# tomneda/DABstar

Hardware: AMD Instinct MI355X
Metric: DAB Mode-I ensembles/s (2.048 MS/s IQ->MSC bytes) per GPU; FIB CRC match % (higher is better)
Workload: dtype f32+i32

## Files before the change

dabstar_amd/csrc/engine.cpp:

```cpp
#include "engine.h"
#include "viterbi_core.h"
#include "fig00.h"
#include <algorithm>
#include <cstddef>
#include <cstring>
#include <map>
#include <string>
#include <tuple>
#include <vector>

int dabx_engine::build_msc_classes()
{
  const EngineDev &d = dev;
  have_fast = false;
  fast = MscFast{};
  for (void *q : fast_allocs) {
    (void)hipFree(q);
    allocs.erase(std::remove(allocs.begin(), allocs.end(), q), allocs.end());
  }
  fast_allocs.clear();
  for (auto &sc : subch_host) sc.fast_class = 0;
  if (d.max_subch <= 0) return 0;
  struct Key { int kbps, prot, shortf, cu; bool operator<(const Key &o) const { return std::tie(kbps, prot, shortf, cu) < std::tie(o.kbps, o.prot, o.shortf, o.cu); } };
  std::map<Key, std::vector<uint32_t>> groups;
// ... 116 lines not shown
{
  if (!cfg || !out || cfg->n_streams <= 0 || cfg->ring_frames < 2 || cfg->max_subch < 0 || cfg->max_subch > MAX_SUBCH ||
      cfg->out_frames < 1 || cfg->soft_bit_type < 1 || cfg->soft_bit_type > 3 || cfg->dc_iq_correction < 0 || cfg->dc_iq_correction > 2 ||
      cfg->viterbi_tie_mode < 0 || cfg->viterbi_tie_mode > 2 || cfg->schedule < 0 || cfg->schedule > 1 ||
      cfg->msc_fast_min_jobs < 0 || cfg->msc_class_min_jobs < 0 || cfg->exact_level_tracker < 0 || cfg->exact_level_tracker > 2 ||
      cfg->acquire_mode < 0 || cfg->acquire_mode > 2) {
    set_error("dabx_create: bad configuration");
    return DABX_E_ARG;
  }
  int rc = need_device_e();
  if (rc) return rc;
  auto *e = new dabx_engine();
  e->cfg = *cfg;
#define H(x) do { hipError_t err__ = (x); if (err__ != hipSuccess) { set_error("HIP error %d (%s) at %s:%d", (int)err__, hipGetErrorString(err__), __FILE__, __LINE__); dabx_destroy(e); return DABX_E_HIP; } } while (0)
  H(hipGetDevice(&e->device));
  int prio_lo = 0, prio_hi = 0;
  (void)hipDeviceGetStreamPriorityRange(&prio_lo, &prio_hi);
  H(hipStreamCreateWithPriority(&e->stream, hipStreamNonBlocking, prio_hi));
  e->ss.a = e->stream;
  if (cfg->schedule == 0) {
    H(hipStreamCreateWithPriority(&e->ss.b, hipStreamNonBlocking, prio_lo));
    H(hipStreamCreateWithPriority(&e->ss.d, hipStreamNonBlocking, prio_hi));
    H(hipEventCreateWithFlags(&e->ss.prep_done, hipEventDisableTiming | hipEventReleaseToDevice));
    H(hipEventCreateWithFlags(&e->ss.msc_done, hipEventDisableTiming | hipEventReleaseToDevice));
    H(hipEventCreateWithFlags(&e->ss.fic_go, hipEventDisableTiming | hipEventReleaseToDevice));
    H(hipEventCreateWithFlags(&e->ss.prep_b_done, hipEventDisableTiming | hipEventReleaseToDevice));
    H(hipEventCreateWithFlags(&e->ss.demap_done, hipEventDisableTiming | hipEventReleaseToDevice));
    H(hipEventCreateWithFlags(&e->ss.sym_done, hipEventDisableTiming | hipEventReleaseToDevice));
    e->ss.fic_on_d = cfg->n_streams < FEW_STREAMS;
    H(hipStreamCreateWithFlags(&e->ingest, hipStreamNonBlocking));
        H(hipStreamCreateWithPriority(&e->ss.q, hipStreamNonBlocking, cfg->exact_level_tracker == 1 ? prio_hi : prio_lo));
    H(hipEventCreateWithFlags(&e->ss.acq_done, hipEventDisableTiming | hipEventReleaseToDevice));
    H(hipEventCreateWithFlags(&e->ss.tail_done, hipEventDisableTiming | hipEventReleaseToDevice));
    H(hipEventCreateWithFlags(&e->ss.acq_a_done, hipEventDisableTiming | hipEventReleaseToDevice));
  }
  if (!e->ingest) H(hipStreamCreateWithFlags(&e->ingest, hipStreamNonBlocking));
  H(hipEventCreateWithFlags(&e->ingest_done, hipEventDisableTiming | hipEventReleaseToDevice));
  e->rd_seen.assign(cfg->n_streams, 0);
  const int S = cfg->n_streams;
  EngineDev &d = e->dev;
  d.n_streams = S; d.max_subch = cfg->max_subch; d.out_frames = cfg->out_frames;
  d.ring_len = cfg->ring_frames * TF;
  d.ring_fmt = e->ring_fmt = ring_fmt;
  d.threshold = cfg->sync_threshold; d.strongest = cfg->sync_strongest;
  d.fic_only = cfg->fic_only; d.capture_soft = cfg->capture_soft; d.tie_mode = cfg->viterbi_tie_mode;
  d.exact_level = cfg->exact_level_tracker == 1;
  d.anchor_level = cfg->exact_level_tracker == 0;
  const DevTables *t;
  if ((rc = get_tables(&t))) { dabx_destroy(e); return rc; }
#define A(x) if ((rc = (x))) { dabx_destroy(e); return rc; }
  A(e->alloc_bytes(&d.iq, (size_t)S * d.ring_len * ring_bytes_per_sample(ring_fmt), false));
  A(e->alloc(&d.wr, S));
  A(e->alloc(&d.ctl, S));
  A(e->alloc(&d.spectra, (size_t)2 * S * 75 * K, false));
  A(e->alloc(&d.fsnap, S));
  A(e->alloc(&d.sym_seq, S));
  A(e->alloc(&d.fic_seq, S));
  A(e->alloc(&d.demap_busy, S));
  A(e->alloc(&d.dciq_state, (size_t)S * 8));
  A(e->alloc(&d.dciq_done, S));
  if (d.exact_level) A(e->alloc(&d.level_pos, S));
  H(hipHostMalloc((void **)&e->locked_host, sizeof(int32_t), hipHostMallocMapped | hipHostMallocCoherent));
  *e->locked_host = 0;
  H(hipHostMalloc((void **)&e->horizon_host, sizeof(unsigned long long) * S, hipHostMallocMapped | hipHostMallocCoherent));
  for (int s = 0; s < S; s++) e->horizon_host[s] = 0;
  e->announcing.assign(S, 0);
  H(hipHostGetDevicePointer((void **)&d.wr_horizon, e->horizon_host, 0));
  H(hipHostGetDevicePointer((void **)&d.locked_count, e->locked_host, 0));
  H(hipHostMalloc((void **)&e->seq_timeouts_host, sizeof(int32_t), hipHostMallocMapped | hipHostMallocCoherent));
  *e->seq_timeouts_host = 0;
  H(hipHostGetDevicePointer((void **)&d.seq_timeouts, e->seq_timeouts_host, 0));
  {
    std::vector<float> st8((size_t)S * 8, 0.0f);
    for (int s_ = 0; s_ < S; s_++) { st8[(size_t)s_ * 8 + 2] = 1.0f; st8[(size_t)s_ * 8 + 3] = 1.0f; }
    H(hipMemcpyAsync(d.dciq_state, st8.data(), sizeof(float) * st8.size(), hipMemcpyHostToDevice, e->stream));
    H(hipStreamSynchronize(e->stream));
  }
  A(e->alloc(&d.nco_tid, (size_t)S * 256));
  A(e->alloc(&d.nco_sym, (size_t)S * 76));
  A(e->alloc(&d.sym_off, (size_t)S * 76));
  A(e->alloc(&e->snap_buf[0], S));
  A(e->alloc(&e->snap_buf[1], S));
  d.snap = e->snap_buf[0];
  A(e->alloc(&d.tii_acc, (size_t)S * TU));
  A(e->alloc(&d.tii_cnt, (size_t)S * 2));
  e->tii.assign((size_t)S, nullptr);
  e->fibdec.assign((size_t)S, nullptr);
  e->fib_frames_fed.assign((size_t)S, 0);
  e->tii_epoch.assign((size_t)S, 0);
  A(e->alloc(&d.cp_part, (size_t)S * 75));
  A(e->alloc(&d.abs_part, (size_t)S * 76));
  A(e->alloc(&d.fic_sym, (size_t)S * 3 * K2));
  A(e->alloc(&d.tdi, (size_t)S * TDI_SLOTS * CIF_BITS));
  A(e->alloc(&d.subch, (size_t)S * std::max(1, d.max_subch)));
  A(e->alloc(&d.fib_out, (size_t)S * d.out_frames * 12 * 32));
  A(e->alloc(&d.fib_crc, (size_t)S * d.out_frames * 12));
  A(e->alloc(&d.frame_pos, (size_t)S * d.out_frames));
  A(e->alloc(&d.frame_start, (size_t)S * d.out_frames));
  if (d.capture_soft) A(e->alloc(&d.soft_cap, (size_t)S * 75 * K2));
  A(e->alloc(&d.sf_info, (size_t)S * std::max(1, d.max_subch) * SF_SLOTS));
  A(demap_alloc(d.demap, S));
  d.demap.soft_type = cfg->soft_bit_type;
  A(launch_demap_init(d.demap, e->stream));
  std::vector<StreamCtl> ctl(S);
  for (auto &c : ctl) {
    memset(&c, 0, sizeof(c));
    c.state = ST_INIT; c.s_level = 0.1f; c.peak_level = -1.0e6f; c.sync_thr = cfg->sync_threshold;
// ... 876 lines not shown
```

dabstar_amd/csrc/ofdm_core.h:

```cpp
#pragma once
#include <hip/hip_runtime.h>
#include "dabx_internal.h"
#include "fft_core.h"
#include "wave_ops.h"

namespace dabx {

__device__ __forceinline__ float cabsf_(float2 z) { return sqrtf(z.x * z.x + z.y * z.y); }
__device__ __forceinline__ float cabsf_level(float2 z) { return __builtin_amdgcn_sqrtf(z.x * z.x + z.y * z.y); }

__device__ __forceinline__ float block_sum(float v, float *red , int tid)
{
  v = wave_sum(v);
  __syncthreads();
  if ((tid & 63) == 0) red[tid >> 6] = v;
  __syncthreads();
  const int nw = blockDim.x >> 6;
  float s = 0.f;
  for (int w = 0; w < nw; w++) s += red[w];
  return s;
}
__device__ __forceinline__ void block_sum2(float &a, float &b, float *red , int tid)
{
  a = wave_sum(a); b = wave_sum(b);
// ... 295 lines not shown
  const float at_axis = mean_level * F_SQRT1_2;
  const float rd = fabsf(b.x) - at_axis, id = fabsf(b.y) - at_axis;
  const float sigma_sq = rd * rd + id * id;
  c.mean_sigma_sq += ALPHA * (sigma_sq - c.mean_sigma_sq);
  float signal_power = c.mean_power - c.null_power;
  if (signal_power <= 0.0f) signal_power = 0.1f;
  const float babs = __builtin_amdgcn_sqrtf(power);
  const float nsr = c.null_power * __builtin_amdgcn_rcpf(signal_power) + 0.7f;
  float w1;
  if (soft_type == 3) {
    w1 = pr_abs;
  } else if (soft_type == 2) {
    w1 = pr_abs * __builtin_amdgcn_rcpf(c.mean_sigma_sq * nsr);
  } else {
    w1 = __builtin_amdgcn_sqrtf(babs * pr_abs) * mean_level * __builtin_amdgcn_rcpf(nsr * (c.mean_sigma_sq * babs));
  }
  const float2 r1 = make_float2(b.x * w1, b.y * w1);
  soft_re = cvt_i16_x86(r1.x * w2);
  soft_im = cvt_i16_x86(r1.y * w2);
  c.prev = x;
  return babs * w1;
}

typedef float v2f __attribute__((ext_vector_type(2)));
typedef int v2i __attribute__((ext_vector_type(2)));
struct DemapPair {
  v2f prev_re, prev_im, integ, mean_power, mean_sigma_sq, null_power;
};
__device__ __forceinline__ v2f v2_rsq(v2f a) { return (v2f){__builtin_amdgcn_rsqf(a.x), __builtin_amdgcn_rsqf(a.y)}; }
__device__ __forceinline__ v2f v2_sqrt(v2f a) { return (v2f){__builtin_amdgcn_sqrtf(a.x), __builtin_amdgcn_sqrtf(a.y)}; }
__device__ __forceinline__ v2f v2_rcp(v2f a) { return (v2f){__builtin_amdgcn_rcpf(a.x), __builtin_amdgcn_rcpf(a.y)}; }
__device__ __forceinline__ v2f v2_abs(v2f a) { return (v2f){fabsf(a.x), fabsf(a.y)}; }
__device__ __forceinline__ v2f v2_fma(v2f a, v2f b, v2f c) { return __builtin_elementwise_fma(a, b, c); }

__device__ __forceinline__ v2f phase_offset_from_diagonal2(v2f y, v2f x, v2f ay, v2f ax)
{
  const v2f mx = (v2f){max3_abs(x.x, y.x, 1.17549435e-38f), max3_abs(x.y, y.y, 1.17549435e-38f)};
  const v2f mnv = (v2f){min_abs(x.x, y.x), min_abs(x.y, y.y)};
  const v2f t = mnv * v2_rcp(mx);
  const v2f z = t * t;
  v2f p = (v2f)(0.0028662257f);
  p = v2_fma(p, z, (v2f)(-0.0161657367f));
  p = v2_fma(p, z, (v2f)(0.0429096138f));
  p = v2_fma(p, z, (v2f)(-0.0752896400f));
  p = v2_fma(p, z, (v2f)(0.1065626393f));
  p = v2_fma(p, z, (v2f)(-0.1420889944f));
  p = v2_fma(p, z, (v2f)(0.1999355085f));
  p = v2_fma(p, z, (v2f)(-0.3333314528f));
  const v2f r = v2_fma(p * z, t, t);
  const v2f u = r - 0.78539816339744830962f, d = ay - ax;
  return (v2f){phase_fold_sign(u.x, d.x, x.x, y.x, t.x), phase_fold_sign(u.y, d.y, x.y, y.y, t.y)};
}

template <int SOFT_TYPE>
__device__ __forceinline__ v2f demap_pair(DemapPair &c, v2f x_re, v2f x_im, v2f rel_f, float clock_err, float w2,
                                          int16_t (&soft_re)[2], int16_t (&soft_im)[2], v2f &power_out, v2f *std_dev_sq = nullptr)
{
  constexpr float ALPHA = 0.005f;
  const float F_PI = 3.14159265358979323846f;
  const float F_RAD_PER_DEG = 0.01745329251994329577f, F_SQRT1_2 = 0.70710678118654752440f;
  const v2f pr_re = c.prev_re, pr_im = c.prev_im;
  const v2f pr_sq = pr_re * pr_re + pr_im * pr_im;
  const v2f pr_inv = v2_rsq(pr_sq);
  const v2f pr_abs = pr_sq * pr_inv;
  const v2f raw_re = (x_re * pr_re + x_im * pr_im) * pr_inv;
  const v2f raw_im = (x_im * pr_re - x_re * pr_im) * pr_inv;
  const v2f phase_err = clock_err * (F_PI / 1024.0f / (float)(K / 2)) * rel_f + c.integ;
  const v2f xx = -phase_err, x2 = xx * xx;
  const v2f sine = xx * (x2 * -0.16034401953220367431640625f + 0.99903142452239990234375f);
  const v2f cosine = 0.9994032382965087890625f + x2 * (x2 * 3.679168224334716796875e-2f + -0.495580852031707763671875f);
  const v2f b_re = raw_re * cosine - raw_im * sine;
  const v2f b_im = raw_re * sine + raw_im * cosine;
  const v2f abs_re = v2_abs(b_re), abs_im = v2_abs(b_im);
  const v2f off = phase_offset_from_diagonal2(b_im, b_re, abs_im, abs_re);
  const v2f integ = c.integ + 0.2f * ALPHA * off;
  const float lim = F_RAD_PER_DEG * 20.0f;
  c.integ = (v2f){__builtin_amdgcn_fmed3f(integ.x, -lim, lim), __builtin_amdgcn_fmed3f(integ.y, -lim, lim)};
  if (std_dev_sq) { v2f sd = *std_dev_sq; sd += ALPHA * (off * off - sd); *std_dev_sq = sd; }
  const v2f power = b_re * b_re + b_im * b_im;
  power_out = power;
  c.mean_power += ALPHA * (power - c.mean_power);
  const v2f mean_level = v2_sqrt(c.mean_power);
  const v2f at_axis = mean_level * F_SQRT1_2;
  const v2f rd = abs_re - at_axis, id = abs_im - at_axis;
  const v2f sigma_sq = rd * rd + id * id;
  c.mean_sigma_sq += ALPHA * (sigma_sq - c.mean_sigma_sq);
  v2f signal_power = c.mean_power - c.null_power;
  signal_power = (signal_power <= 0.0f) ? (v2f)(0.1f) : signal_power;
  const v2f babs = v2_sqrt(power);
  const v2f nsr = c.null_power * v2_rcp(signal_power) + 0.7f;
  v2f w1;
  if (SOFT_TYPE == 3) w1 = pr_abs;
  else if (SOFT_TYPE == 2) w1 = pr_abs * v2_rcp(c.mean_sigma_sq * nsr);
  else w1 = v2_sqrt(babs * pr_abs) * mean_level * v2_rcp(nsr * (c.mean_sigma_sq * babs));
  const v2f r1_re = b_re * w1, r1_im = b_im * w1;
  const v2f s_re = r1_re * w2, s_im = r1_im * w2;
  cvt4_i16_x86(s_re.x, s_re.y, s_im.x, s_im.y, soft_re[0], soft_re[1], soft_im[0], soft_im[1]);
  c.prev_re = x_re; c.prev_im = x_im;
  return babs * w1;
}

__device__ __forceinline__ float demap_w2(float mean_value, int soft_type)
{
  return (soft_type == 1 ? -100.0f : -140.0f) * __builtin_amdgcn_rcpf(mean_value);
}

__device__ __forceinline__ float mpa_weight(int k)
{
  const float a = 0.005f / (float)K;
  return a * __expf((float)(K - 1 - k) * -3.2552135e-6f);
}
__device__ __forceinline__ float mpa_decay() { return 0.99501247f; }
__device__ __forceinline__ float mpa_decay_n(int n_sym) { return __expf((float)n_sym * (float)K * -3.2552135e-6f); }
__device__ __forceinline__ float snr_db_from(float mean_power_all, float null_sum)
{
  const float kMinNoisePower = (1.0f / 32767.0f) * (1.0f / 32767.0f);
  if (null_sum == 0.0f) null_sum = kMinNoisePower * (float)K;
  const float noise = null_sum / (float)K;
  float snr = (mean_power_all - noise) / noise;
// ... 27 lines not shown
```

dabstar_amd/csrc/pipeline.h:

```cpp
#pragma once
#include "dabx_internal.h"
#include "ring_fmt.h"

namespace dabx {

#ifndef DABX_MSC_BATCH
#define DABX_MSC_BATCH 7
#endif
constexpr int MSC_SLOTS = DABX_MSC_BATCH > 7 ? 64 : 32;
constexpr int MSC_BATCH_FRAMES = DABX_MSC_BATCH;
constexpr int SF_SLOTS = 16;
constexpr int ACQ_NEED = 20 * TU + 50 + (TF + 1) + (TN + 50 + 21) + 64;
constexpr int FRAME_NEED = TF + 2 * TU;
constexpr int FEW_STREAMS = 48;

enum StreamState : int32_t { ST_INIT = 0, ST_WAIT_SYNC = 1, ST_EVAL_SYNC = 2 };

struct StreamCtl {
  unsigned long long rd;
  unsigned long long sym0_pos;
  long long cif_no;
  long long msc_done_cif;
  long long frames;
  int32_t state;
// ... 4 lines not shown
  float sync_thr;
  int32_t sample_count;
  int32_t start_index;
  int32_t correction;
  int32_t frame_ok;
  int32_t phase_sym1;
  int32_t f_frame;
  int32_t fic_ratio;
  int32_t cif_count;
  int32_t fic_errors, fic_bits, fic_block;
  int32_t fic_status_errors, fic_status_bits;
  float mer_db;
  float snr_db;
  long long fib_ok, fib_total, sync_lost;
  float head_abs_a, head_abs_b;
  int32_t np_sel;
  int32_t pad_;
  long long level_margin;
  unsigned long long lvl_anchor_pos, lvl_approx_pos;
  float lvl_anchor_S;
  int32_t pad3_;
  long long lvl_rewalks, lvl_unanchored;
  long long lvl_healed;
  unsigned long long lvl_hist_pos[16];
  float lvl_hist_S[16];
};
constexpr int LVL_HIST = 16;

struct SubchDev {
  int32_t cu_start, cu_size, kbps, prot_level, short_form, dab_plus;
  int32_t nbits;
  int32_t active;
  int32_t fast_class, pad_;
  const uint16_t *map;
  long long start_cif;
  long long cif_out;
  int32_t blocks_in_buf, sf_sync;
  long long sf_count;
  long long sf_ok, sf_fail, rs_corr, rs_fail, fc_corr, au_ok, au_bad;
  long long move_cif;
  int32_t prev_cu_start, pad2_;
};
#ifdef __HIPCC__
__device__ __forceinline__ int msc_move_thr(const SubchDev &sc, long long r)
{
  const long long t = sc.move_cif - r + 16;
  return t <= 0 ? 0 : (t >= 16 ? 16 : (int)t);
}
#endif

struct BatchSnap { long long msc_done, cif_no; };
struct FrameSnap { long long cif0; float clock_err; int32_t frame_ok, np_sel, pad_; };

struct EngineDev {
  int32_t n_streams, max_subch, out_frames;
  int32_t ring_len;
  float threshold;
  int32_t strongest, fic_only, capture_soft;
  int32_t exact_level;
  int32_t anchor_level;
  unsigned long long *wr_horizon;
  unsigned long long *level_pos;
  int32_t *locked_count;
  int32_t tie_mode;
  int32_t msc_stride;
  int32_t sf_stride;
  int32_t vit_stride;
  void *iq;
  int32_t ring_fmt;
  unsigned long long *wr;
  StreamCtl *ctl;
  DemapDev demap;
  float2 *spectra;
  FrameSnap *fsnap;
  int32_t *demap_busy;
  float *dciq_state;
  unsigned long long *dciq_done;
  int32_t parity;
  int32_t s0;
  int32_t flag_sync;
  uint32_t step_seq;
  uint32_t *sym_seq, *fic_seq;
  int32_t *seq_timeouts;
  double2 *nco_tid;
  double2 *nco_sym;
  int32_t *sym_off;
  float2 *cp_part;
  float *abs_part;
  uint8_t *fic_sym;
  uint8_t *tdi;
  uint32_t *vit_scratch;
  SubchDev *subch;
  uint8_t *fib_out;
  uint8_t *fib_crc;
  long long *frame_pos;
  int32_t *frame_start;
  uint8_t *msc_out;
  uint8_t *sf_out;
  dabx_superframe_info *sf_info;
  int16_t *soft_cap;
  BatchSnap *snap;
  float2 *tii_acc;
  int32_t *tii_cnt;
};

struct DeliverDev {
  uint8_t *slab;
  const unsigned long long *layout_off;
  const int32_t *subch_id;
  long long *frames_done;
  long long *cif_done, *sf_done;
  dabx_chunk_header hdr;
  hipEvent_t lf_done;
};

constexpr int MSC_MAX_CLASSES = DABX_MSC_FAST_CLASSES;
struct MscClass {
  int n_in, nbits;
  int n_pairs;
  const uint16_t *map2;
  const uint32_t *pairs;
  uint32_t *inT[2];
  uint2 *decT;
};
struct MscFast {
  int n_cls;
// ... 164 lines not shown
```

dabstar_amd/csrc/pipeline.hip:

```cpp
#include <type_traits>
#include "pipeline.h"
#include "packet_core.h"
#include "pad_core.h"
#include "mot_core.h"
#include "carousel_core.h"
#include <algorithm>
#include "ofdm_core.h"
#include "viterbi_core.h"
#include "fec_core.h"
#include "acq_walk.h"
#include "level_par.h"
#include "fig00.h"

namespace dabx {

__device__ __forceinline__ void front_prio() { __builtin_amdgcn_s_setprio(3); }

template <class T> __device__ __forceinline__ T uniform_load(const T *p)
{
  typedef unsigned Raw __attribute__((ext_vector_type(sizeof(T) / 4)));
  const Raw raw = *(const __attribute__((address_space(4))) Raw *)(const void *)p;
  return __builtin_bit_cast(T, raw);
}

// ... 724 lines not shown
  FftTwiddles tw;
  fft_load_twiddles(tw, t.twiddle, tid);
  const uint4 kk4 = reinterpret_cast<const uint4 *>(t.bin_to_slot8)[tid];
  const unsigned kkw[4] = {kk4.x, kk4.y, kk4.z, kk4.w};
  const unsigned rd_lo = t.carrier_slot_rd[tid];
  for (;;) {
    float2 cb0 = Fmt::cvt(nx[0]), ca0 = Fmt::cvt(nx[1]), cb1 = Fmt::cvt(nx[2]), ca1 = Fmt::cvt(nx[3]);
    float2 v[8];
#pragma unroll
    for (int u = 0; u < 8; u++) v[u] = Fmt::cvt(nx[4 + u]);
    const double2 base_now = nco_base;
    const int l_next = l + (int)gridDim.x;
    if (l_next < 75) {
      off = uniform_load(e.sym_off + (size_t)s * 76 + l_next);
      nco_base = uniform_load(e.nco_sym + (size_t)s * 76 + l_next);
      request(off);
    }
    asm volatile("" ::: "memory");
    float cre = 0.f, cim = 0.f, asum = 0.f;
    cre += ca0.x * cb0.x + ca0.y * cb0.y;
    cim += ca0.y * cb0.x - ca0.x * cb0.y;
    asum += cabsf_level(cb0);
    if (two) {
      cre += ca1.x * cb1.x + ca1.y * cb1.y;
      cim += ca1.y * cb1.x - ca1.x * cb1.y;
      asum += cabsf_level(cb1);
    }
    Nco nco;
    nco.init_from(base_now, nco_step, nco_t);
#pragma unroll
    for (int u = 0; u < 8; u++) {
      const float2 x = v[u];
      asum += cabsf_level(x);
      v[u] = nco.mix(x);
      nco.step();
    }
    cre = wave_sum(cre); cim = wave_sum(cim); asum = wave_sum(asum);
    if ((tid & 63) == 0) { red3[0][tid >> 6] = cre; red3[1][tid >> 6] = cim; red3[2][tid >> 6] = asum; }
    fft2048_regs<false>(v, lds, tw, tid);
    if (tid == 0) {
      float r[3];
#pragma unroll
      for (int q = 0; q < 3; q++) { float a = 0.f; for (int w = 0; w < 4; w++) a += red3[q][w]; r[q] = a; }
      e.cp_part[(size_t)s * 75 + l] = make_float2(r[0], r[1]); e.abs_part[(size_t)s * 76 + l] = r[2];
    }
#pragma unroll
    for (int u = 0; u < 8; u++) {
      unsigned kw = kkw[u >> 1];
      if (RF != RING_CF32) asm volatile("" : "+v"(kw));
      const int kk = (int)(int16_t)(kw >> (16 * (u & 1)));
      if (kk >= 0) lds[kk] = v[u];
    }
    __syncthreads();
    float2 *dst = e.spectra + (((size_t)e.parity * e.n_streams + s) * 75 + l) * K;
#pragma unroll
    for (int u = 0; u < K / 256; u++) {
      typedef float sym_f2 __attribute__((ext_vector_type(2)));
      const float2 q = lds[((tid + 256 * u) & ~15) | ((rd_lo >> (4 * u)) & 15u)];
      sym_f2 qv; qv.x = q.x; qv.y = q.y;
      __builtin_nontemporal_store(qv, reinterpret_cast<sym_f2 *>(dst + tid + 256 * u));
    }
    if (l_next >= 75) break;
    l = l_next;
    __syncthreads();
  }
}

__device__ __forceinline__ void seq_publish(uint32_t *p, uint32_t seq)
{
  __syncthreads();
  if (threadIdx.x == 0) {
    __threadfence();
    __hip_atomic_store(p, seq, __ATOMIC_RELEASE, __HIP_MEMORY_SCOPE_AGENT);
  }
}
__device__ __forceinline__ void seq_wait(const uint32_t *p, uint32_t seq, int32_t *timeouts)
{
  if (threadIdx.x == 0) {
    int spins = 0;
    while ((int32_t)(__hip_atomic_load(p, __ATOMIC_ACQUIRE, __HIP_MEMORY_SCOPE_AGENT) - seq) < 0) {
      __builtin_amdgcn_s_sleep(8);
      if (++spins > (8 << 20)) {
        if (timeouts) __hip_atomic_fetch_add(timeouts, 1, __ATOMIC_RELAXED, __HIP_MEMORY_SCOPE_SYSTEM);
        break;
      }
    }
  }
  __syncthreads();
  __builtin_amdgcn_fence(__ATOMIC_ACQUIRE, "agent");
}
__global__ void k_sym_publish(EngineDev e)
{
  const int s = blockIdx.x * blockDim.x + threadIdx.x;
  if (s < e.n_streams) __hip_atomic_store(e.sym_seq + s, e.step_seq, __ATOMIC_RELEASE, __HIP_MEMORY_SCOPE_AGENT);
}

constexpr int DEMAP_Q = 2, DEMAP_THREADS = K / DEMAP_Q, DEMAP_NP = DEMAP_Q / 2;
constexpr int DEMAP_NOUT = (K2 / 4) / DEMAP_THREADS;
constexpr int TILE_PLANE = 196;
__device__ __forceinline__ float2 demap_ld_spec(const float2 *p)
{
  typedef float dm_f2 __attribute__((ext_vector_type(2)));
  const dm_f2 q = __builtin_nontemporal_load(reinterpret_cast<const dm_f2 *>(p));
  return make_float2(q.x, q.y);
}
template <int SOFT_TYPE, bool SAT, bool WHOLE = false, bool MER = false>
__device__ __forceinline__ void demap_frame_body(EngineDev &e, const DevTables &t, const int l0, const int l1)
{
  if (l0 == 0) __builtin_amdgcn_s_setprio(3); else __builtin_amdgcn_s_setprio(1);
  __shared__ __attribute__((aligned(16))) float red[32];
  __shared__ __attribute__((aligned(16))) uint8_t tile[2][16 * TILE_PLANE];
  __shared__ v2f sd_lds[MER ? DEMAP_NP * DEMAP_THREADS : 1];
  const int s = blockIdx.x + e.s0, tid = threadIdx.x;
  StreamCtl &c = e.ctl[s];
  if (l0 == 0 && e.flag_sync) seq_wait(e.sym_seq + s, e.step_seq, e.seq_timeouts);
  FrameSnap fs;
  if (l0 == 0) {
    fs.cif0 = c.cif_no; fs.clock_err = c.clock_err; fs.frame_ok = c.frame_ok; fs.np_sel = c.np_sel; fs.pad_ = 0;
    if (tid == 0) {
      e.fsnap[s] = fs;
      if (fs.frame_ok && e.demap_busy) __hip_atomic_store(&e.demap_busy[s], 1, __ATOMIC_RELAXED, __HIP_MEMORY_SCOPE_AGENT);
    }
  } else fs = e.fsnap[s];
  if (!fs.frame_ok) {
    if (l0 == 0 && e.flag_sync) seq_publish(e.fic_seq + s, e.step_seq);
    return;
  }
  DemapDev &d = e.demap;
  const float *null_power = fs.np_sel ? d.null_power2 : d.null_power;
  const float2 *spectra = e.spectra + (size_t)e.parity * e.n_streams * 75 * K;
  DemapPair cr[DEMAP_NP];
  v2f rel_f[DEMAP_NP], wk[DEMAP_NP], pacc[DEMAP_NP];
#pragma unroll
  for (int q = 0; q < DEMAP_Q; q++) {
    const int k = tid + DEMAP_THREADS * q, p = q >> 1, h = q & 1;
    const int bin = t.perm_bin[k];
    rel_f[p][h] = (float)(K / 2 - t.perm_rel[k]);
    const float2 pr = l0 == 0 ? d.phase_ref[(size_t)s * TU + bin] : spectra[((size_t)s * 75 + (l0 - 1)) * K + k];
    cr[p].prev_re[h] = pr.x; cr[p].prev_im[h] = pr.y;
    cr[p].integ[h] = d.integ[(size_t)s * K + k];
    cr[p].mean_power[h] = d.mean_power[(size_t)s * K + k];
    cr[p].mean_sigma_sq[h] = d.mean_sigma[(size_t)s * K + k];
    cr[p].null_power[h] = null_power[(size_t)s * TU + bin];
    wk[p][h] = mpa_weight(k);
    pacc[p][h] = 0.0f;
    if constexpr (MER) sd_lds[p * DEMAP_THREADS + tid][h] = d.std_dev[(size_t)s * K + k];
  }
  float mean_value = d.mean_value[s], mpa = d.mean_power_all[s];
  const float ce = fs.clock_err;
  const long long cif0 = (long long)(((unsigned long long)(unsigned)__builtin_amdgcn_readfirstlane((int)((unsigned long long)fs.cif0 >> 32)) << 32) |
                                     (unsigned)__builtin_amdgcn_readfirstlane((int)(unsigned)fs.cif0));
  uint8_t *fic = e.fic_sym + (size_t)s * 3 * K2;
  uint8_t *tdi = e.tdi + (size_t)s * TDI_SLOTS * CIF_BITS;
  int16_t *cap = e.capture_soft ? e.soft_cap + (size_t)s * 75 * K2 : nullptr;
  float2 xn[DEMAP_Q];
  const float2 *xp = spectra + ((size_t)s * 75 + l0) * K + tid + (DEMAP_Q / 2) * DEMAP_THREADS;
#pragma unroll
  for (int q = 0; q < DEMAP_Q; q++) xn[q] = demap_ld_spec(xp + (q - DEMAP_Q / 2) * DEMAP_THREADS);
  static_assert(DEMAP_Q % 2 == 0 && K % DEMAP_Q == 0 && (K2 / 4) % DEMAP_THREADS == 0 && DEMAP_THREADS % 64 == 0, "tile <-> thread mapping below");
  int tpos[2 * DEMAP_Q];
#pragma unroll
  for (int q = 0; q < DEMAP_Q; q++) {
    const int k = tid + DEMAP_THREADS * q;
    tpos[2 * q] = (k & 15) * TILE_PLANE + (k >> 4);
    tpos[2 * q + 1] = ((K + k) & 15) * TILE_PLANE + ((K + k) >> 4);
  }
  auto symbol = [&](const int l, auto par) {
    constexpr int PAR = decltype(par)::value;
    if (l < 74) xp += K;
    const int m = l - 3, cif = m / 18, blk = m % 18;
    const float w2 = demap_w2(mean_value, SOFT_TYPE);
    uint8_t *tl = tile[PAR];
    float2 xc[DEMAP_Q];
#pragma unroll
    for (int q = 0; q < DEMAP_Q; q++) { xc[q] = xn[q]; xn[q] = demap_ld_spec(xp + (q - DEMAP_Q / 2) * DEMAP_THREADS); }
    float part = 0.f;
#pragma unroll
    for (int p = 0; p < DEMAP_NP; p++) {
      int16_t sr[2], si[2];
      v2f pw;
      const v2f mag = demap_pair<SOFT_TYPE>(cr[p], (v2f){xc[2 * p].x, xc[2 * p + 1].x}, (v2f){xc[2 * p].y, xc[2 * p + 1].y}, rel_f[p], ce, w2, sr, si, pw,
                                            MER ? &sd_lds[p * DEMAP_THREADS + tid] : nullptr);
      part = p == 0 ? mag.x + mag.y : part + (mag.x + mag.y);
      pacc[p] = pacc[p] * mpa_decay() + pw;
#pragma unroll
      for (int h = 0; h < 2; h++) {
        const int q = 2 * p + h;
        tl[tpos[2 * q]] = SAT ? soft_to_sym_sat(sr[h]) : soft_to_sym(sr[h]);
        tl[tpos[2 * q + 1]] = SAT ? soft_to_sym_sat(si[h]) : soft_to_sym(si[h]);
        if (cap) { const int k = tid + DEMAP_THREADS * q; cap[(size_t)l * K2 + k] = sr[h]; cap[(size_t)l * K2 + K + k] = si[h]; }
      }
    }
    {
      float *rp = red + 16 * PAR;
      const float pw_sum = wave_sum(part);
      if ((tid & 63) == 0) rp[tid >> 6] = pw_sum;
      __syncthreads();
      float sum = 0.f;
      if constexpr (DEMAP_THREADS / 64 == 12) {
        const v2f *rp2 = reinterpret_cast<const v2f *>(rp);
        const v2f a = ((rp2[0] + rp2[1]) + (rp2[2] + rp2[3])) + (rp2[4] + rp2[5]);
        sum = a.x + a.y;
      } else {
#pragma unroll
        for (int w = 0; w < DEMAP_THREADS / 64; w++) sum += rp[w];
      }
      mean_value = sum * (1.0f / (float)K);
    }
#pragma unroll
    for (int j = 0; j < DEMAP_NOUT; j++) {
      const int dwi = tid + DEMAP_THREADS * j;
      if (l < 3) {
        uint32_t v = 0;
#pragma unroll
        for (int b = 0; b < 4; b++) { const int i = 4 * dwi + b; v |= (uint32_t)tl[(i & 15) * TILE_PLANE + (i >> 4)] << (8 * b); }
        reinterpret_cast<uint32_t *>(fic + l * K2)[dwi] = v;
      } else {
        const int out_plane = dwi / 48, out_dw = dwi - out_plane * 48;
        const uint32_t v = *reinterpret_cast<const uint32_t *>(tl + out_plane * TILE_PLANE + 4 * out_dw);
        static_assert(K2 % 16 == 0, "a symbol is a whole number of positions in every plane");
        uint8_t *const tdi_thr = tdi + (size_t)out_plane * (CIF_BITS / 16) + 4 * out_dw;
        const size_t uoff = (size_t)((cif0 + cif) & (TDI_SLOTS - 1)) * CIF_BITS + (size_t)blk * (K2 / 16);
        *reinterpret_cast<uint32_t *>(tdi_thr + uoff) = v;
      }
    }
  };
  auto run = [&](int a, int b) {
    int l = a;
    for (; l + 1 < b; l += 2) { symbol(l, std::integral_constant<int, 0>{}); symbol(l + 1, std::integral_constant<int, 1>{}); }
    if (l < b) symbol(l, std::integral_constant<int, 0>{});
  };
  constexpr bool whole_frame_flagged = WHOLE;
  if constexpr (WHOLE) {
    run(0, 3);
    seq_publish(e.fic_seq + s, e.step_seq);
    run(3, l1);
  } else run(l0, l1);
#pragma unroll
  for (int q = 0; q < DEMAP_Q; q++) {
    const int k = tid + DEMAP_THREADS * q, p = q >> 1, h = q & 1;
    d.integ[(size_t)s * K + k] = cr[p].integ[h];
    d.mean_power[(size_t)s * K + k] = cr[p].mean_power[h];
    d.mean_sigma[(size_t)s * K + k] = cr[p].mean_sigma_sq[h];
  }
  if constexpr (MER) {
    float sd = 0.f;
#pragma unroll
    for (int q = 0; q < DEMAP_Q; q++) {
      const float v = sd_lds[(q >> 1) * DEMAP_THREADS + tid][q & 1];
      d.std_dev[(size_t)s * K + tid + DEMAP_THREADS * q] = v;
      sd += v;
    }
    if (l1 == 75) {
      sd = block_sum(sd, red, tid);
      if (tid == 0) c.mer_db = mer_db_from(sd);
      __syncthreads();
    }
  }
  float ns = cr[0].null_power.x + cr[0].null_power.y, wsum = wk[0].x * pacc[0].x + wk[0].y * pacc[0].y;
#pragma unroll
  for (int p = 1; p < DEMAP_NP; p++) { ns += cr[p].null_power.x + cr[p].null_power.y; wsum += wk[p].x * pacc[p].x + wk[p].y * pacc[p].y; }
  block_sum2w(ns, wsum, red, tid);
  if (tid == 0) {
    mpa = mpa * mpa_decay_n(l1 - l0) + wsum;
    d.mean_value[s] = mean_value; d.mean_power_all[s] = mpa;
    if (l1 == 75) c.snr_db = snr_db_from(mpa, ns);
  }
  if (l0 == 0 && e.flag_sync && !whole_frame_flagged) seq_publish(e.fic_seq + s, e.step_seq);
  if (l1 == 75 && e.demap_busy) {
    __syncthreads();
    if (tid == 0) __hip_atomic_store(&e.demap_busy[s], 0, __ATOMIC_RELEASE, __HIP_MEMORY_SCOPE_AGENT);
  }
}

template <int SOFT_TYPE, bool SAT, bool MER>
__global__ __launch_bounds__(DEMAP_THREADS, 6) void k_demap_frame6(EngineDev e, DevTables t, int l0, int l1) { demap_frame_body<SOFT_TYPE, SAT, false, MER>(e, t, l0, l1); }
template <int SOFT_TYPE, bool SAT, bool MER>
__global__ __launch_bounds__(DEMAP_THREADS) void k_demap_fic(EngineDev e, DevTables t) { demap_frame_body<SOFT_TYPE, SAT, false, MER>(e, t, 0, 3); }
template <int SOFT_TYPE, bool SAT, bool MER>
__global__ __launch_bounds__(DEMAP_THREADS) void k_demap_whole(EngineDev e, DevTables t) { demap_frame_body<SOFT_TYPE, SAT, true, MER>(e, t, 0, 75); }

struct SrcFic {
  const uint8_t *sym;
  const uint16_t *map;
  typedef ushort4 Key;
  struct Raw { uint8_t a, b, c, d; };
  __device__ Key key(int t) const { return *reinterpret_cast<const ushort4 *>(map + 4 * t); }
  __device__ uint8_t ld(uint16_t idx) const { return sym[idx == PUNCT ? 0 : idx]; }
  __device__ Raw raw(Key m) const { return {ld(m.x), ld(m.y), ld(m.z), ld(m.w)}; }
  __device__ static int cv(uint8_t v, uint16_t idx) { return vit_sym_from_u8(idx == PUNCT ? (uint8_t)127 : v); }
  __device__ VitSyms syms(Raw r, Key m) const { return {cv(r.a, m.x), cv(r.b, m.y), cv(r.c, m.z), cv(r.d, m.w)}; }
};

__global__ __launch_bounds__(256) void k_fic_frame(EngineDev e, DevTables t, int first, int count)
{
  front_prio();
  __shared__ __attribute__((aligned(16))) char wtab[4][VIT_BLK * 16];
  __shared__ uint32_t fibw[4][24];
  __shared__ uint32_t raw[4][32];
  __shared__ uint8_t crc_ok[12];
  __shared__ uint32_t encw[4][26];
  __shared__ int ber_err[4];
  __shared__ uint16_t s_crc[256];
  const int s = blockIdx.x, wave = threadIdx.x >> 6, lane = threadIdx.x & 63;
  StreamCtl &c = e.ctl[s];
  if (e.flag_sync && first == 0 && count == 4) seq_wait(e.fic_seq + s, e.step_seq, e.seq_timeouts);
  if (!c.frame_ok) return;
  s_crc[threadIdx.x] = t.crc_ccitt[threadIdx.x];
  const int fic = first + wave;
  if (wave < count) {
    SrcFic src{e.fic_sym + (size_t)s * 3 * K2 + fic * FIC_IN, t.fic_map};
    uint32_t *dec = e.vit_scratch + ((size_t)s * 4 + fic) * (size_t)e.vit_stride;
    const VitLaneConst k = vit_lane_const(lane);
    if (e.tie_mode == 2) vit_forward<2>(src, FIC_OUT + 6, wtab[wave], dec, lane, k);
    else if (e.tie_mode) vit_forward<1>(src, FIC_OUT + 6, wtab[wave], dec, lane, k);
    else vit_forward<0>(src, FIC_OUT + 6, wtab[wave], dec, lane, k);
    __builtin_amdgcn_fence(__ATOMIC_RELEASE, "workgroup");
// ... 561 lines not shown
  hipLaunchKernelGGL(k_msc_inject, dim3((unsigned)(((size_t)n_cifs * CIF_BITS + 255) / 256)), dim3(256), 0, st, e, stream, soft_dev, n_cifs, first);
  DABX_HIP(hipGetLastError());
  return 0;
}
int launch_msc_advance(const EngineDev &e, const int32_t *counts_dev, hipStream_t st)
{
  hipLaunchKernelGGL(k_msc_advance, dim3((e.n_streams + 255) / 256), dim3(256), 0, st, e, counts_dev);
  DABX_HIP(hipGetLastError());
  return 0;
}

__global__ void k_fic_inject(EngineDev e, int s, const int16_t *soft)
{
  const int i = blockIdx.x * blockDim.x + threadIdx.x;
  if (i < 3 * K2) e.fic_sym[(size_t)s * 3 * K2 + i] = soft_to_sym_mode(soft[i], e.tie_mode);
}
__global__ void k_fic_present(EngineDev e, const int32_t *present)
{
  const int s = blockIdx.x * blockDim.x + threadIdx.x;
  if (s < e.n_streams) e.ctl[s].frame_ok = present[s] ? 1 : 0;
}
__global__ void k_fic_advance(EngineDev e, const int32_t *present)
{
  const int s = blockIdx.x * blockDim.x + threadIdx.x;
  if (s < e.n_streams && present[s]) e.ctl[s].frames += 1;
}
int launch_fic_inject(const EngineDev &e, int stream, const int16_t *soft_dev, hipStream_t st)
{
  hipLaunchKernelGGL(k_fic_inject, dim3(3 * K2 / 256), dim3(256), 0, st, e, stream, soft_dev);
  DABX_HIP(hipGetLastError());
  return 0;
}
int launch_fic_decode(const EngineDev &e_in, const int32_t *present_dev, hipStream_t st)
{
  const DevTables *t;
  int rc = get_tables(&t);
  if (rc) return rc;
  EngineDev e = e_in;
  e.flag_sync = 0;
  const dim3 grid((e.n_streams + 255) / 256);
  hipLaunchKernelGGL(k_fic_present, grid, dim3(256), 0, st, e, present_dev);
  hipLaunchKernelGGL(k_fic_frame, dim3(e.n_streams), dim3(256), 0, st, e, *t, 0, 4);
  hipLaunchKernelGGL(k_fic_advance, grid, dim3(256), 0, st, e, present_dev);
  DABX_HIP(hipGetLastError());
  return 0;
}

__global__ __launch_bounds__(256) void k_demap_inject(EngineDev e, DevTables t, int s, const float2 *spec, const float2 *null_fft, float clock_err, int np_sel)
{
  const int l = blockIdx.x, tid = threadIdx.x;
  if (l == 0) {
    for (int i = tid; i < TU; i += 256) e.demap.phase_ref[(size_t)s * TU + i] = spec[i];
  } else if (l <= 75) {
    float2 *dst = e.spectra + (((size_t)e.parity * e.n_streams + s) * 75 + (l - 1)) * K;
    for (int k = tid; k < K; k += 256) dst[k] = spec[(size_t)l * TU + t.perm_bin[k]];
  } else {
    if (null_fft) {
      float *np = (np_sel ? e.demap.null_power2 : e.demap.null_power) + (size_t)s * TU;
      for (int k = tid; k < K; k += 256) { const int bin = t.perm_bin[k]; np[bin] = null_power_next(np[bin], null_fft[bin]); }
    }
    if (tid == 0) { e.ctl[s].clock_err = clock_err; e.ctl[s].np_sel = np_sel; }
  }
}
int launch_demap_inject(const EngineDev &e_in, int parity, int stream, const float2 *spec_dev, const float2 *null_dev, float clock_err, int np_sel, hipStream_t st)
{
  const DevTables *t;
  int rc = get_tables(&t);
  if (rc) return rc;
  EngineDev e = e_in;
  e.parity = parity;
  hipLaunchKernelGGL(k_demap_inject, dim3(77), dim3(256), 0, st, e, *t, stream, spec_dev, null_dev, clock_err, np_sel);
  DABX_HIP(hipGetLastError());
  return 0;
}
int launch_demap_frame(const EngineDev &e_in, unsigned step_count, const int32_t *present_dev, int schedule, hipStream_t st)
{
  const DevTables *t;
  int rc = get_tables(&t);
  if (rc) return rc;
  EngineDev e = e_in;
  e.parity = (int)(step_count & 1u);
  e.step_seq = step_count;
  e.flag_sync = 0;
  hipLaunchKernelGGL(k_fic_present, dim3((e.n_streams + 255) / 256), dim3(256), 0, st, e, present_dev);
  if (schedule == 0) {
    DABX_DEMAP_DISPATCH(k_demap_frame6, dim3(e.n_streams), dim3(DEMAP_THREADS), 0, st, e, *t, 0, 75);
  } else if (schedule == 1) {
    DABX_DEMAP_DISPATCH(k_demap_fic, dim3(e.n_streams), dim3(DEMAP_THREADS), 0, st, e, *t);
    DABX_DEMAP_DISPATCH(k_demap_frame6, dim3(e.n_streams), dim3(DEMAP_THREADS), 0, st, e, *t, 3, 75);
  } else {
    DABX_DEMAP_DISPATCH(k_demap_whole, dim3(e.n_streams), dim3(DEMAP_THREADS), 0, st, e, *t);
  }
  DABX_HIP(hipGetLastError());
  return 0;
}

__global__ void k_commit(unsigned long long *wr, int n_streams, int stream, unsigned long long n)
{
  const int i = blockIdx.x * blockDim.x + threadIdx.x;
  if (i < n_streams && (stream < 0 || i == stream)) wr[i] += n;
}
int launch_commit(const EngineDev &e, int stream, unsigned long long n, hipStream_t st)
{
  hipLaunchKernelGGL(k_commit, dim3((e.n_streams + 255) / 256), dim3(256), 0, st, e.wr, e.n_streams, stream, n);
  DABX_HIP(hipGetLastError());
  return 0;
}

// ... 2 lines not shown
```

Measured before the change: 564,100.

## Interleave spectra carrier pairs into float4 layout for single vector loads in demap

Changes the intermediate spectra buffer from per-carrier float2 to a float4 layout that packs the two carriers each demap thread handles (k and k+K/2) in re/re/im/im order. The FFT writer, the injection kernel and the demap loader all switch to 128-bit accesses, so each demap symbol needs one vector load instead of two. The next-symbol prefetch is now placed inside demap_pair through a hook, after the raw differential product. A few register-pressure tweaks are also added: mean_power_all is loaded late and tid goes through an asm barrier. The cost is a more complex indexing scheme that ties the layout to DEMAP_Q == 2.

```diff
diff --git a/dabstar_amd/csrc/engine.cpp b/dabstar_amd/csrc/engine.cpp
--- a/dabstar_amd/csrc/engine.cpp
+++ b/dabstar_amd/csrc/engine.cpp
@@ -192,7 +192,7 @@
   A(e->alloc_bytes(&d.iq, (size_t)S * d.ring_len * ring_bytes_per_sample(ring_fmt), false));
   A(e->alloc(&d.wr, S));
   A(e->alloc(&d.ctl, S));
-  A(e->alloc(&d.spectra, (size_t)2 * S * 75 * K, false));
+  A(e->alloc(&d.spectra, spectra_count(S), false));
   A(e->alloc(&d.fsnap, S));
   A(e->alloc(&d.sym_seq, S));
   A(e->alloc(&d.fic_seq, S));
diff --git a/dabstar_amd/csrc/ofdm_core.h b/dabstar_amd/csrc/ofdm_core.h
--- a/dabstar_amd/csrc/ofdm_core.h
+++ b/dabstar_amd/csrc/ofdm_core.h
@@ -371,9 +371,11 @@
   return (v2f){phase_fold_sign(u.x, d.x, x.x, y.x, t.x), phase_fold_sign(u.y, d.y, x.y, y.y, t.y)};
 }
 
-template <int SOFT_TYPE>
+struct DemapNoHook { __device__ __forceinline__ void operator()() const {} };
+template <int SOFT_TYPE, class PrevDead = DemapNoHook>
 __device__ __forceinline__ v2f demap_pair(DemapPair &c, v2f x_re, v2f x_im, v2f rel_f, float clock_err, float w2,
-                                          int16_t (&soft_re)[2], int16_t (&soft_im)[2], v2f &power_out, v2f *std_dev_sq = nullptr)
+                                          int16_t (&soft_re)[2], int16_t (&soft_im)[2], v2f &power_out, v2f *std_dev_sq = nullptr,
+                                          PrevDead prev_dead = PrevDead())
 {
   constexpr float ALPHA = 0.005f;
   const float F_PI = 3.14159265358979323846f;
@@ -384,6 +386,7 @@
   const v2f pr_abs = pr_sq * pr_inv;
   const v2f raw_re = (x_re * pr_re + x_im * pr_im) * pr_inv;
   const v2f raw_im = (x_im * pr_re - x_re * pr_im) * pr_inv;
+  prev_dead();
   const v2f phase_err = clock_err * (F_PI / 1024.0f / (float)(K / 2)) * rel_f + c.integ;
   const v2f xx = -phase_err, x2 = xx * xx;
   const v2f sine = xx * (x2 * -0.16034401953220367431640625f + 0.99903142452239990234375f);
diff --git a/dabstar_amd/csrc/pipeline.h b/dabstar_amd/csrc/pipeline.h
--- a/dabstar_amd/csrc/pipeline.h
+++ b/dabstar_amd/csrc/pipeline.h
@@ -80,6 +80,13 @@
 struct BatchSnap { long long msc_done, cif_no; };
 struct FrameSnap { long long cif0; float clock_err; int32_t frame_ok, np_sel, pad_; };
 
+constexpr int SPEC_PAIRS = K / 2;
+constexpr size_t spectra_count(int n_streams) { return (size_t)2 * n_streams * 75 * SPEC_PAIRS; }
+#ifdef __HIPCC__
+__host__ __device__ inline size_t spectra_sym(int parity, int n_streams, int s, int l) { return (((size_t)parity * n_streams + s) * 75 + l) * SPEC_PAIRS; }
+__host__ __device__ inline float4 spectra_elem(float2 a, float2 b) { return make_float4(a.x, b.x, a.y, b.y); }
+#endif
+
 struct EngineDev {
   int32_t n_streams, max_subch, out_frames;
   int32_t ring_len;
@@ -99,7 +106,7 @@
   unsigned long long *wr;
   StreamCtl *ctl;
   DemapDev demap;
-  float2 *spectra;
+  float4 *spectra;
   FrameSnap *fsnap;
   int32_t *demap_busy;
   float *dciq_state;
diff --git a/dabstar_amd/csrc/pipeline.hip b/dabstar_amd/csrc/pipeline.hip
--- a/dabstar_amd/csrc/pipeline.hip
+++ b/dabstar_amd/csrc/pipeline.hip
@@ -800,13 +800,15 @@
       if (kk >= 0) lds[kk] = v[u];
     }
     __syncthreads();
-    float2 *dst = e.spectra + (((size_t)e.parity * e.n_streams + s) * 75 + l) * K;
-#pragma unroll
-    for (int u = 0; u < K / 256; u++) {
-      typedef float sym_f2 __attribute__((ext_vector_type(2)));
-      const float2 q = lds[((tid + 256 * u) & ~15) | ((rd_lo >> (4 * u)) & 15u)];
-      sym_f2 qv; qv.x = q.x; qv.y = q.y;
-      __builtin_nontemporal_store(qv, reinterpret_cast<sym_f2 *>(dst + tid + 256 * u));
+    float4 *dst = e.spectra + spectra_sym(e.parity, e.n_streams, s, l);
+#pragma unroll
+    for (int u = 0; u < SPEC_PAIRS / 256; u++) {
+      typedef float sym_f4 __attribute__((ext_vector_type(4)));
+      const float2 qa = lds[((tid + 256 * u) & ~15) | ((rd_lo >> (4 * u)) & 15u)];
+      const float2 qb = lds[((tid + 256 * u + SPEC_PAIRS) & ~15) | ((rd_lo >> (4 * (u + SPEC_PAIRS / 256))) & 15u)];
+      const float4 q = spectra_elem(qa, qb);
+      sym_f4 qv; qv.x = q.x; qv.y = q.y; qv.z = q.z; qv.w = q.w;
+      __builtin_nontemporal_store(qv, reinterpret_cast<sym_f4 *>(dst + tid + 256 * u));
     }
     if (l_next >= 75) break;
     l = l_next;
@@ -846,11 +848,10 @@
 constexpr int DEMAP_Q = 2, DEMAP_THREADS = K / DEMAP_Q, DEMAP_NP = DEMAP_Q / 2;
 constexpr int DEMAP_NOUT = (K2 / 4) / DEMAP_THREADS;
 constexpr int TILE_PLANE = 196;
-__device__ __forceinline__ float2 demap_ld_spec(const float2 *p)
-{
-  typedef float dm_f2 __attribute__((ext_vector_type(2)));
-  const dm_f2 q = __builtin_nontemporal_load(reinterpret_cast<const dm_f2 *>(p));
-  return make_float2(q.x, q.y);
+typedef float dm_f4 __attribute__((ext_vector_type(4)));
+__device__ __forceinline__ dm_f4 demap_ld_spec(const float4 *p)
+{
+  return __builtin_nontemporal_load(reinterpret_cast<const dm_f4 *>(p));
 }
 template <int SOFT_TYPE, bool SAT, bool WHOLE = false, bool MER = false>
 __device__ __forceinline__ void demap_frame_body(EngineDev &e, const DevTables &t, const int l0, const int l1)
@@ -876,15 +877,18 @@
   }
   DemapDev &d = e.demap;
   const float *null_power = fs.np_sel ? d.null_power2 : d.null_power;
-  const float2 *spectra = e.spectra + (size_t)e.parity * e.n_streams * 75 * K;
+  static_assert(DEMAP_Q == 2 && DEMAP_THREADS == SPEC_PAIRS, "one carrier pair per thread");
+  const float4 *spectra = e.spectra + spectra_sym(e.parity, e.n_streams, s, 0);
   DemapPair cr[DEMAP_NP];
   v2f rel_f[DEMAP_NP], wk[DEMAP_NP], pacc[DEMAP_NP];
+  dm_f4 xprev = {0.f, 0.f, 0.f, 0.f};
+  if (l0 > 0) xprev = *reinterpret_cast<const dm_f4 *>(spectra + (size_t)(l0 - 1) * SPEC_PAIRS + tid);
 #pragma unroll
   for (int q = 0; q < DEMAP_Q; q++) {
     const int k = tid + DEMAP_THREADS * q, p = q >> 1, h = q & 1;
     const int bin = t.perm_bin[k];
     rel_f[p][h] = (float)(K / 2 - t.perm_rel[k]);
-    const float2 pr = l0 == 0 ? d.phase_ref[(size_t)s * TU + bin] : spectra[((size_t)s * 75 + (l0 - 1)) * K + k];
+    const float2 pr = l0 == 0 ? d.phase_ref[(size_t)s * TU + bin] : make_float2(xprev[h], xprev[2 + h]);
     cr[p].prev_re[h] = pr.x; cr[p].prev_im[h] = pr.y;
     cr[p].integ[h] = d.integ[(size_t)s * K + k];
     cr[p].mean_power[h] = d.mean_power[(size_t)s * K + k];
@@ -894,17 +898,15 @@
     pacc[p][h] = 0.0f;
     if constexpr (MER) sd_lds[p * DEMAP_THREADS + tid][h] = d.std_dev[(size_t)s * K + k];
   }
-  float mean_value = d.mean_value[s], mpa = d.mean_power_all[s];
+  float mean_value = d.mean_value[s];
   const float ce = fs.clock_err;
   const long long cif0 = (long long)(((unsigned long long)(unsigned)__builtin_amdgcn_readfirstlane((int)((unsigned long long)fs.cif0 >> 32)) << 32) |
                                      (unsigned)__builtin_amdgcn_readfirstlane((int)(unsigned)fs.cif0));
   uint8_t *fic = e.fic_sym + (size_t)s * 3 * K2;
   uint8_t *tdi = e.tdi + (size_t)s * TDI_SLOTS * CIF_BITS;
   int16_t *cap = e.capture_soft ? e.soft_cap + (size_t)s * 75 * K2 : nullptr;
-  float2 xn[DEMAP_Q];
-  const float2 *xp = spectra + ((size_t)s * 75 + l0) * K + tid + (DEMAP_Q / 2) * DEMAP_THREADS;
-#pragma unroll
-  for (int q = 0; q < DEMAP_Q; q++) xn[q] = demap_ld_spec(xp + (q - DEMAP_Q / 2) * DEMAP_THREADS);
+  const float4 *xp = spectra + (size_t)l0 * SPEC_PAIRS + tid;
+  dm_f4 xn = demap_ld_spec(xp);
   static_assert(DEMAP_Q % 2 == 0 && K % DEMAP_Q == 0 && (K2 / 4) % DEMAP_THREADS == 0 && DEMAP_THREADS % 64 == 0, "tile <-> thread mapping below");
   int tpos[2 * DEMAP_Q];
 #pragma unroll
@@ -915,20 +917,19 @@
   }
   auto symbol = [&](const int l, auto par) {
     constexpr int PAR = decltype(par)::value;
-    if (l < 74) xp += K;
+    if (l < 74) xp += SPEC_PAIRS;
     const int m = l - 3, cif = m / 18, blk = m % 18;
     const float w2 = demap_w2(mean_value, SOFT_TYPE);
     uint8_t *tl = tile[PAR];
-    float2 xc[DEMAP_Q];
-#pragma unroll
-    for (int q = 0; q < DEMAP_Q; q++) { xc[q] = xn[q]; xn[q] = demap_ld_spec(xp + (q - DEMAP_Q / 2) * DEMAP_THREADS); }
+    const dm_f4 xc = xn;
+    auto fetch = [&]() { xn = demap_ld_spec(xp); };
     float part = 0.f;
 #pragma unroll
     for (int p = 0; p < DEMAP_NP; p++) {
       int16_t sr[2], si[2];
       v2f pw;
-      const v2f mag = demap_pair<SOFT_TYPE>(cr[p], (v2f){xc[2 * p].x, xc[2 * p + 1].x}, (v2f){xc[2 * p].y, xc[2 * p + 1].y}, rel_f[p], ce, w2, sr, si, pw,
-                                            MER ? &sd_lds[p * DEMAP_THREADS + tid] : nullptr);
+      const v2f mag = demap_pair<SOFT_TYPE>(cr[p], (v2f){xc.x, xc.y}, (v2f){xc.z, xc.w}, rel_f[p], ce, w2, sr, si, pw,
+                                            MER ? &sd_lds[p * DEMAP_THREADS + tid] : nullptr, fetch);
       part = p == 0 ? mag.x + mag.y : part + (mag.x + mag.y);
       pacc[p] = pacc[p] * mpa_decay() + pw;
 #pragma unroll
@@ -984,9 +985,11 @@
     seq_publish(e.fic_seq + s, e.step_seq);
     run(3, l1);
   } else run(l0, l1);
+  int tid_st = tid;
+  asm volatile("" : "+v"(tid_st));
 #pragma unroll
   for (int q = 0; q < DEMAP_Q; q++) {
-    const int k = tid + DEMAP_THREADS * q, p = q >> 1, h = q & 1;
+    const int k = tid_st + DEMAP_THREADS * q, p = q >> 1, h = q & 1;
     d.integ[(size_t)s * K + k] = cr[p].integ[h];
     d.mean_power[(size_t)s * K + k] = cr[p].mean_power[h];
     d.mean_sigma[(size_t)s * K + k] = cr[p].mean_sigma_sq[h];
@@ -1010,7 +1013,7 @@
   for (int p = 1; p < DEMAP_NP; p++) { ns += cr[p].null_power.x + cr[p].null_power.y; wsum += wk[p].x * pacc[p].x + wk[p].y * pacc[p].y; }
   block_sum2w(ns, wsum, red, tid);
   if (tid == 0) {
-    mpa = mpa * mpa_decay_n(l1 - l0) + wsum;
+    const float mpa = d.mean_power_all[s] * mpa_decay_n(l1 - l0) + wsum;
     d.mean_value[s] = mean_value; d.mean_power_all[s] = mpa;
     if (l1 == 75) c.snr_db = snr_db_from(mpa, ns);
   }
@@ -1678,8 +1681,8 @@
   if (l == 0) {
     for (int i = tid; i < TU; i += 256) e.demap.phase_ref[(size_t)s * TU + i] = spec[i];
   } else if (l <= 75) {
-    float2 *dst = e.spectra + (((size_t)e.parity * e.n_streams + s) * 75 + (l - 1)) * K;
-    for (int k = tid; k < K; k += 256) dst[k] = spec[(size_t)l * TU + t.perm_bin[k]];
+    float4 *dst = e.spectra + spectra_sym(e.parity, e.n_streams, s, l - 1);
+    for (int j = tid; j < SPEC_PAIRS; j += 256) dst[j] = spectra_elem(spec[(size_t)l * TU + t.perm_bin[j]], spec[(size_t)l * TU + t.perm_bin[j + SPEC_PAIRS]]);
   } else {
     if (null_fft) {
       float *np = (np_sel ? e.demap.null_power2 : e.demap.null_power) + (size_t)s * TU;
```

Result: no change. 561,600 (-0.4%).
